# JokerJohn/Cloud_Map_Evaluation

Measured on AMD Instinct MI355X. Metric: Mpts/sec full metric suite (CD+MME+AWD) on 50M-pt pair, higher is better.
Workload: dtype f64

## Files before the change

cloud_map_evaluation_amd/csrc/me_api.hip:

```cpp
#include <cmath>
#include <cstring>

#include "me_internal.hpp"
#include "me_stat.hpp"

static std::string g_create_error;

hipEvent_t me_ctx::get_event() {
    if (!event_pool.empty()) {
        hipEvent_t e = event_pool.back();
        event_pool.pop_back();
        return e;
    }
    hipEvent_t e = nullptr;
    (void) hipEventCreate(&e);
    return e;
}

void me_ctx::timer_begin(const char *name) {
    if (!timers_on) return;
    Pending p;
    p.name = name;
    p.a = get_event();
    p.b = get_event();
// ... 26 lines not shown
__global__ void __launch_bounds__(64) k_mail(const unsigned char *__restrict__ src, unsigned char *__restrict__ dst, unsigned int bytes) {
    if (((reinterpret_cast<size_t>(src) | reinterpret_cast<size_t>(dst) | bytes) & 7u) == 0) {
        for (unsigned int i = threadIdx.x; i < bytes / 8; i += 64)
            reinterpret_cast<unsigned long long *>(dst)[i] = reinterpret_cast<const unsigned long long *>(src)[i];
    } else {
        for (unsigned int i = threadIdx.x; i < bytes; i += 64) dst[i] = src[i];
    }
}

int copy_h2d(me_ctx *ctx, void *dst_device, const void *src_host, size_t bytes) {
    if (bytes == 0) return ME_OK;
    ME_CHECK(ctx, hipMemcpyAsync(dst_device, src_host, bytes, hipMemcpyHostToDevice, ctx->stream));
    return ME_OK;
}

int copy_d2h(me_ctx *ctx, void *dst_host, const void *src_device, size_t bytes) {
    if (bytes == 0) return ME_OK;
    ME_CHECK(ctx, hipMemcpyAsync(dst_host, src_device, bytes, hipMemcpyDeviceToHost, ctx->stream));
    ME_CHECK(ctx, hipStreamSynchronize(ctx->stream));
    return ME_OK;
}

int mail_post(me_ctx *ctx, void *host_dst, const void *dev_src, size_t bytes) {
    if (bytes == 0) return ME_OK;
    if (!ctx->mail_h) {
        void *h = nullptr, *d = nullptr;
        ME_CHECK(ctx, hipHostMalloc(&h, kMailBytes, hipHostMallocMapped));
        ME_CHECK(ctx, hipHostGetDevicePointer(&d, h, 0));
        ctx->mail_h = static_cast<unsigned char *>(h);
        ctx->mail_d = static_cast<unsigned char *>(d);
    }
    const size_t off = (ctx->mail_used + 15) & ~(size_t) 15;
    if (off + bytes > kMailBytes) return copy_d2h(ctx, host_dst, dev_src, bytes);
    hipLaunchKernelGGL(k_mail, dim3(1), dim3(64), 0, ctx->stream, static_cast<const unsigned char *>(dev_src), ctx->mail_d + off,
                       (unsigned int) bytes);
    ctx->mail_pending.push_back({host_dst, off, bytes});
    ctx->mail_used = off + bytes;
    return ME_OK;
}

int mail_sync(me_ctx *ctx) {
    const hipError_t e = hipStreamSynchronize(ctx->stream);
    if (e == hipSuccess)
        for (const auto &m : ctx->mail_pending) std::memcpy(m.host, ctx->mail_h + m.off, m.bytes);
    ctx->mail_pending.clear();
    ctx->mail_used = 0;
    ME_CHECK(ctx, e);
    return ME_OK;
}

void mail_drop(me_ctx *ctx) {
    ctx->mail_pending.clear();
    ctx->mail_used = 0;
}

int need_single_gpu_cloud(me_ctx *ctx, int slot, const char *who) {
    if (slot < 0 || slot > 1) return ctx->fail(ME_ERR_ARG, std::string(who) + ": bad slot");
    Cloud &c = ctx->cloud[slot];
    if (ctx->shard_world != 1 || ctx->slab.axis >= 0 || c.slab.axis >= 0)
        return ctx->fail(ME_ERR_ARG, std::string(who) + ": single GPU only (no slab or shard mode)");
    if (!c.uploaded) return ctx->fail(ME_ERR_STATE, std::string(who) + ": cloud not uploaded");
    return ME_OK;
}
}

extern "C" {

int me_version(void) { return 100; }

static int stream_priority_for(bool main_lane) {
    int least = 0, greatest = 0;
    (void) hipDeviceGetStreamPriorityRange(&least, &greatest);
    return main_lane ? greatest : least;
}

me_ctx *me_create(int device, int flags) {
    int count = 0;
    hipError_t e = hipGetDeviceCount(&count);
    if (e != hipSuccess || count <= 0) {
        g_create_error = std::string("me_create: no HIP device available (") + hipGetErrorString(e) +
                         "); libmapeval_hip has no CPU fallback";
        return nullptr;
    }
    if (device < 0 || device >= count) {
        g_create_error = "me_create: device ordinal out of range";
        return nullptr;
    }
    e = hipSetDevice(device);
    if (e != hipSuccess) {
        g_create_error = std::string("me_create: hipSetDevice: ") + hipGetErrorString(e);
        return nullptr;
    }
    me_ctx *ctx = new me_ctx();
    ctx->device = device;
    ctx->borrow_device_input = (flags & ME_FLAG_BORROW_DEVICE_INPUT) != 0;
    ctx->morton_order = (flags & ME_FLAG_MORTON_ORDER) != 0;
    e = hipStreamCreateWithPriority(&ctx->stream, hipStreamNonBlocking, stream_priority_for(true));
    if (e != hipSuccess) {
        g_create_error = std::string("me_create: hipStreamCreate: ") + hipGetErrorString(e);
        delete ctx;
        return nullptr;
    }
    return ctx;
}

me_ctx *me_twin(me_ctx *ctx) {
    if (!ctx) return nullptr;
    if (ctx->is_twin) return ctx;
    if (ctx->twin) return ctx->twin;
    if (hipSetDevice(ctx->device) != hipSuccess) {
        ctx->fail(ME_ERR_HIP, "me_twin: hipSetDevice failed");
        return nullptr;
    }
    me_ctx *t = new me_ctx();
    t->device = ctx->device;
    t->is_twin = true;
    t->cloud.p[0] = ctx->cloud.p[0];
    t->cloud.p[1] = ctx->cloud.p[1];
    t->shard_rank = ctx->shard_rank;
    t->shard_world = ctx->shard_world;
    t->borrow_device_input = ctx->borrow_device_input;
    t->morton_order = ctx->morton_order;
    t->slab = ctx->slab;
    t->vox_hint = ctx->vox_hint;
    if (hipStreamCreateWithPriority(&t->stream, hipStreamNonBlocking, stream_priority_for(false)) != hipSuccess) {
        delete t;
        ctx->fail(ME_ERR_HIP, "me_twin: hipStreamCreate failed");
        return nullptr;
    }
    ctx->twin = t;
    return t;
}

void me_destroy(me_ctx *ctx) {
    if (!ctx) return;
    if (ctx->is_twin) return;
    if (ctx->suite_worker && ctx->suite_worker_free) {
        ctx->suite_worker_free(ctx->suite_worker);
        ctx->suite_worker = nullptr;
    }
    if (ctx->twin) {
        me_ctx *t = ctx->twin;
        ctx->twin = nullptr;
        t->is_twin = false;
        me_destroy(t);
    }
    (void) hipSetDevice(ctx->device);
    (void) hipStreamSynchronize(ctx->stream);
    for (auto &p : ctx->pending) {
        (void) hipEventDestroy(p.a);
        (void) hipEventDestroy(p.b);
    }
    for (auto e : ctx->event_pool) (void) hipEventDestroy(e);
    if (ctx->suite_event) (void) hipEventDestroy(static_cast<hipEvent_t>(ctx->suite_event));
    if (ctx->stream) (void) hipStreamDestroy(ctx->stream);
    if (ctx->mail_h) (void) hipHostFree(ctx->mail_h);
    delete ctx;
}

const char *me_last_error(me_ctx *ctx) { return ctx ? ctx->err.c_str() : g_create_error.c_str(); }

int me_set_shard(me_ctx *ctx, int rank, int world) {
    if (!ctx) return ME_ERR_ARG;
    if (world < 1 || rank < 0 || rank >= world) return ctx->fail(ME_ERR_ARG, "me_set_shard: need 0 <= rank < world");
    ctx->shard_rank = rank;
    ctx->shard_world = world;
    if (ctx->twin) {
        ctx->twin->shard_rank = rank;
        ctx->twin->shard_world = world;
    }
    return ME_OK;
}

int me_upload_cloud(me_ctx *ctx, int slot, const double *xyz_host, int64_t n, const double *T, double cell_size) {
    if (!ctx) return ME_ERR_ARG;
    return me::cloud_upload(ctx, slot, xyz_host, false, n, T, cell_size);
}

int me_upload_cloud_device(me_ctx *ctx, int slot, const double *xyz_device, int64_t n, const double *T, double cell_size) {
    if (!ctx) return ME_ERR_ARG;
    return me::cloud_upload(ctx, slot, xyz_device, true, n, T, cell_size);
}

int me_upload_slab_device(me_ctx *ctx, int slot, const double *xyz_device, int64_t n, double cell_size) {
    if (!ctx) return ME_ERR_ARG;
    if (ctx->slab.axis < 0) return ctx->fail(ME_ERR_STATE, "me_upload_slab_device: call me_set_slab first");
    return me::cloud_upload(ctx, slot, xyz_device, true, n, nullptr, cell_size, true);
}

int64_t me_cloud_size(me_ctx *ctx, int slot) {
    if (!ctx || slot < 0 || slot > 1 || !ctx->cloud[slot].uploaded) return -1;
    return ctx->cloud[slot].n;
}

int me_download_cloud(me_ctx *ctx, int slot, double *xyz_host) {
    if (!ctx) return ME_ERR_ARG;
    if (slot < 0 || slot > 1 || !xyz_host) return ctx->fail(ME_ERR_ARG, "me_download_cloud: bad argument");
    me::Cloud &c = ctx->cloud[slot];
    if (!c.uploaded) return ctx->fail(ME_ERR_STATE, "cloud not uploaded");
    ME_CHECK(ctx, hipSetDevice(ctx->device));
    ME_TRY(me::copy_d2h(ctx, xyz_host, c.xyz.p, (size_t) c.n * 24));
    ME_CHECK(ctx, hipStreamSynchronize(ctx->stream));
    return ME_OK;
}

int me_voxel_downsample(me_ctx *ctx, int slot, double voxel_size, int64_t *n_out) {
    if (!ctx) return ME_ERR_ARG;
    long long n = 0;
// ... 556 lines not shown
```

cloud_map_evaluation_amd/csrc/me_index.hip:

```cpp
#include <cmath>
#include <cstdlib>
#include <cstring>

#include "me_internal.hpp"
#include "me_vox_rows.hpp"

namespace me {

struct Mat4 {
    double m[16];
};

__global__ void k_transform(double *__restrict__ xyz, long long n, Mat4 T) {
    const long long i = (long long) blockIdx.x * blockDim.x + threadIdx.x;
    if (i >= n) return;
    const double x = xyz[3 * i], y = xyz[3 * i + 1], z = xyz[3 * i + 2];
    double h[4];
#pragma unroll
    for (int r = 0; r < 4; ++r) h[r] = ((T.m[4 * r] * x + T.m[4 * r + 1] * y) + T.m[4 * r + 2] * z) + T.m[4 * r + 3];
    xyz[3 * i] = h[0] / h[3];
    xyz[3 * i + 1] = h[1] / h[3];
    xyz[3 * i + 2] = h[2] / h[3];
}

// ... 727 lines not shown
    int L = 0;
    long long off = 0;
    for (int k = nn_shift; k <= kMortonBits; ++k) {
        if (L >= kMaxLevels) return ctx->fail(ME_ERR_ARG, "octree deeper than the level table (cloud extent / cell size too large)");
        v.count[L] = c.level_unique[k];
        v.off[L] = off;
        off += v.count[L] + 1;
        ++L;
        if (c.level_unique[k] == 1) break;
    }
    v.n_levels = L;
    ME_CHECK(ctx, c.oct_nodes.ensure((size_t) (off + kFan) * sizeof(ONode)));
    ME_CHECK(ctx, hipMemsetAsync(c.oct_nodes.as<ONode>() + off, 0, kFan * sizeof(ONode), ctx->stream));
    ME_CHECK(ctx, c.oct_pbegin.ensure((size_t) (off + kFan + 1) * 4));
    ME_CHECK(ctx, hipMemsetAsync(c.oct_pbegin.as<unsigned int>() + off, 0, (kFan + 1) * 4, ctx->stream));
    v.nodes = c.oct_nodes.as<ONode>();
    v.pbegin = c.oct_pbegin.as<unsigned int>();
    ONode *nodes = c.oct_nodes.as<ONode>();
    unsigned int *pbeg = c.oct_pbegin.as<unsigned int>();
    hipLaunchKernelGGL(k_oct_leaves, dim3(blocks_of((v.count[0] + 1) * 8)), dim3(256), 0, ctx->stream, c.sp.as<SPoint>(),
                       c.nn_grid.cell_start, v.count[0], n, nodes, pbeg);
    DevBuf &ca = ctx->tmp[2], &cb = ctx->tmp[3], &pos = ctx->tmp[1], &begin = ctx->tmp[4];
    const unsigned long long *cur = c.nn_grid.cell_code;
    for (int l = 0; l + 1 < L; ++l) {
        const long long nc = v.count[l], np = v.count[l + 1];
        if (nc <= kOctTopMax) {
            ME_CHECK(ctx, begin.ensure((size_t) (np + 1) * 4));
            ME_CHECK(ctx, ca.ensure((size_t) np * 8));
            ME_CHECK(ctx, cb.ensure((size_t) np * 8));
            unsigned long long *first = (cur == ca.as<unsigned long long>()) ? cb.as<unsigned long long>() : ca.as<unsigned long long>();
            unsigned long long *second = (first == ca.as<unsigned long long>()) ? cb.as<unsigned long long>() : ca.as<unsigned long long>();
            if (small_top)
                hipLaunchKernelGGL((k_oct_top<256>), dim3(1), dim3(256), 0, ctx->stream, nodes, pbeg, v, l, cur, first, second,
                                   begin.as<unsigned int>());
            else
                hipLaunchKernelGGL((k_oct_top<1024>), dim3(1), dim3(1024), 0, ctx->stream, nodes, pbeg, v, l, cur, first, second,
                                   begin.as<unsigned int>());
            break;
        }
        ME_CHECK(ctx, pos.ensure((size_t) nc * 4));
        ME_CHECK(ctx, begin.ensure((size_t) (np + 1) * 4));
        DevBuf &nxt = (l % 2 == 0) ? ca : cb;
        ME_CHECK(ctx, nxt.ensure((size_t) np * 8));
        ME_TRY(cell_start_ranks(ctx, cur, nc, 3, pos.as<unsigned int>()));
        hipLaunchKernelGGL(k_cell_scatter, dim3(blocks_of(nc)), dim3(256), 0, ctx->stream, cur, pos.as<unsigned int>(), nc, 3,
                           nxt.as<unsigned long long>(), begin.as<unsigned int>());
        hipLaunchKernelGGL(k_oct_up, dim3(blocks_of(np + 1)), dim3(256), 0, ctx->stream, nodes + v.off[l], nc,
                           begin.as<unsigned int>(), np, nodes + v.off[l + 1], pbeg + v.off[l], pbeg + v.off[l + 1]);
        cur = nxt.as<unsigned long long>();
    }
    return ME_OK;
}

int cloud_build_index(me_ctx *ctx, int slot, double cell_size) {
    Cloud &c = ctx->cloud[slot];
    ME_TRACE_POINT(ctx, slot == 0 ? "cloud_build_index(est): enter" : "cloud_build_index(gt): enter");
    if (!c.uploaded) return ctx->fail(ME_ERR_STATE, "cloud not uploaded");
    ME_CHECK(ctx, hipSetDevice(ctx->device));
    c.cell_size_req = cell_size;
    const long long n = c.n;
    double extent = 0;
    for (int d = 0; d < 3; ++d) extent = std::fmax(extent, c.bbox_hi[d] - c.bbox_lo[d]);
    if (!(cell_size > 0)) cell_size = (extent > 0 ? extent / 128.0 : 1.0);
    const double cell_h = cell_size * (1.0 + 0x1p-20);
    for (int d = 0; d < 3; ++d) c.origin[d] = std::floor(c.bbox_lo[d] / cell_h) * cell_h;
    extent = 0;
    for (int d = 0; d < 3; ++d) extent = std::fmax(extent, c.bbox_hi[d] - c.origin[d]);
    const double ncell = std::floor(extent / cell_h) + 1.0;
    int bits_cell = 1;
    while ((double) (1LL << bits_cell) < ncell && bits_cell <= kMortonBits) ++bits_cell;
    if (bits_cell > kMortonBits)
        return ctx->fail(ME_ERR_ARG, "cell size too small for the cloud extent (needs > 2^21 cells per axis)");
    c.shift = kMortonBits - bits_cell;
    c.cell_h = cell_h;
    c.fine_h = std::ldexp(cell_h, -c.shift);
    c.index_valid = false;
    c.mme_have = false;
    c.lg_have = false;
#ifdef ME_AB
    c.mme_feat_valid = false;
#endif
    c.nn_ref_slot = -1;
    ctx->cloud[1 - slot].nn_ref_slot = -1;

    DevBuf &codes_in = ctx->tmp[0], &iota = ctx->tmp[1], &perm = ctx->tmp[2];
    ME_CHECK(ctx, codes_in.ensure((size_t) n * 8));
    ME_CHECK(ctx, iota.ensure((size_t) n * 4));
    ME_CHECK(ctx, perm.ensure((size_t) n * 4));
    ME_CHECK(ctx, c.codes.ensure((size_t) n * 8));
    ME_CHECK(ctx, c.sp.ensure((size_t) n * sizeof(SPoint)));
    constexpr int sort_depth = ME_TUNE_SORT_DEPTH;
    const int hilbert = ctx->morton_order ? 0 : 1;
    int idx_bits = 1;
    while ((1LL << idx_bits) < n) ++idx_bits;
    constexpr int pack_allowed = ME_TUNE_SORT_PACK;
    int sort_min_level = std::max(0, c.shift - std::max(0, sort_depth));
    int pack_bits = 0;
    const bool pairs_hinted = c.sort_pairs_hint && c.hint_n == n && c.hint_shift == c.shift && c.hint_cell_h == cell_h;
    if (!pairs_hinted) c.sort_pairs_hint = false;
    if (pack_allowed && !pairs_hinted) {
        const int lvl_max = std::max(sort_min_level, c.shift - std::min(std::max(0, sort_depth), 1));
        int lvl = sort_min_level;
        while (lvl < lvl_max && 3 * (kMortonBits - lvl) + idx_bits > 64) ++lvl;
        if (3 * (kMortonBits - lvl) + idx_bits <= 64) {
            sort_min_level = lvl;
            pack_bits = idx_bits;
        }
    }
    const bool depth_cut = pack_bits > 0 && sort_min_level > std::max(0, c.shift - std::max(0, sort_depth));
#ifdef ME_DBG_INDEX
    std::fprintf(stderr, "[index slot %d] n=%lld cell_h=%.17g origin=(%.17g %.17g %.17g) bbox_lo=(%.17g %.17g %.17g) shift=%d sort_min_level=%d pack_bits=%d hinted=%d\n", slot, n, cell_h,
                 c.origin[0], c.origin[1], c.origin[2], c.bbox_lo[0], c.bbox_lo[1], c.bbox_lo[2], c.shift, sort_min_level, pack_bits, (int) pairs_hinted);
#endif
    if (pack_bits > 0) ME_CHECK(ctx, perm.ensure((size_t) n * 8));
    {
        TimerScope ts(ctx, "morton");
        hipLaunchKernelGGL(k_morton, dim3(blocks_of(n)), dim3(256), 0, ctx->stream, c.xyz.as<double>(), n, c.origin[0],
                           c.origin[1], c.origin[2], c.fine_h, sort_min_level, hilbert, pack_bits, codes_in.as<unsigned long long>(),
                           iota.as<unsigned int>());
    }
    if (pack_bits > 0)
        ME_TRY(sort_keys_u64(ctx, codes_in.as<unsigned long long>(), perm.as<unsigned long long>(), n, pack_bits,
                             pack_bits + 3 * (kMortonBits - sort_min_level)));
    else
        ME_TRY(sort_pairs_u64_u32(ctx, codes_in.as<unsigned long long>(), c.codes.as<unsigned long long>(),
                                  iota.as<unsigned int>(), perm.as<unsigned int>(), n, 3 * sort_min_level, 63));
    if (ctx->sort_hook) ctx->sort_hook(ctx->sort_hook_arg, ctx->stream);
    VoxPack vp{};
    c.vox_rec_valid = false;
    const bool fuse_vox = ME_TUNE_VOX_ONEPASS && ctx->vox_hint > 0 && vox_make_pack(c, ctx->vox_hint, n, vp);
    const long long rec_cap = vox_record_capacity(n);
    if (fuse_vox) {
        ME_CHECK(ctx, c.vox_rec_key.ensure((size_t) rec_cap * 8));
        ME_CHECK(ctx, c.vox_rec_n.ensure((size_t) rec_cap * 4));
        ME_CHECK(ctx, c.vox_rec_s.ensure((size_t) rec_cap * 8 * kVoxRec));
        ME_CHECK(ctx, c.vox_rec_cnt.ensure(kVoxCounterBytes));
        ME_CHECK(ctx, hipMemsetAsync(c.vox_rec_key.p, 0xFF, (size_t) rec_cap * 8, ctx->stream));
        ME_CHECK(ctx, hipMemsetAsync(c.vox_rec_cnt.p, 0, kVoxCounterBytes, ctx->stream));
    }
    {
        TimerScope ts(ctx, "gather");
#define ME_LAUNCH_GATHER(VOX_, PER_)                                                                                                     \
    hipLaunchKernelGGL((k_gather<VOX_, PER_>), dim3(blocks_of(n, 256 * PER_)), dim3(256), 0, ctx->stream, c.xyz.as<double>(),            \
                       pack_bits > 0 ? (const unsigned int *) nullptr : perm.as<unsigned int>(),                                       \
                       pack_bits > 0 ? perm.as<unsigned long long>() : (const unsigned long long *) nullptr,                           \
                       pack_bits > 0 ? ((1ULL << pack_bits) - 1ULL) : 0ULL, n, c.origin[0], c.origin[1], c.origin[2], c.fine_h,        \
                       c.sp.as<SPoint>(), c.codes.as<unsigned long long>(), vp, c.slab, c.vox_rec_key.as<unsigned long long>(),        \
                       c.vox_rec_n.as<int>(), c.vox_rec_s.as<double>(), c.vox_rec_cnt.as<unsigned int>(), (unsigned int) ((n + 63) / 64), \
                       (unsigned int) vox_region_size(n))
        if (fuse_vox) ME_LAUNCH_GATHER(true, kGatherPerVox);
        else ME_LAUNCH_GATHER(false, kGatherPer);
#undef ME_LAUNCH_GATHER
    }
    if (fuse_vox) {
        c.vox_rec_valid = true;
        c.vox_rec_cap = rec_cap;
        c.vox_rec_pack = vp;
    }
    {
        TimerScope ts(ctx, "cells");
        const int nblk = (int) ((n + kCellChunk - 1) / kCellChunk);
        ME_CHECK(ctx, ctx->red.ensure(64 * 8 + (size_t) (nblk + 2) * 4 * (2 + kHistLevels)));
        unsigned long long *d_hist = ctx->red.as<unsigned long long>();
        unsigned int *d_boff = reinterpret_cast<unsigned int *>(d_hist + 64), *d_bcnt = d_boff + (nblk + 2), *d_bhist = d_bcnt + (nblk + 2);
        ME_CHECK(ctx, hipMemsetAsync(d_hist, 0, 32 * 8, ctx->stream));
        hipLaunchKernelGGL(k_level_hist_rows, dim3((unsigned int) nblk), dim3(256), 0, ctx->stream, c.codes.as<unsigned long long>(), n, d_bhist);
        hipLaunchKernelGGL(k_block_counts<true>, dim3(blocks_of(nblk + 1)), dim3(256), 0, ctx->stream, d_bhist, nblk, c.shift, d_bcnt, d_hist);
        ME_TRY(exclusive_scan_u32(ctx, d_bcnt, d_boff, nblk + 1));
        unsigned long long h_hist[32];
        {
            MailGuard mg(ctx);
            ME_TRY(mail_post(ctx, h_hist, d_hist, sizeof(h_hist)));
            ME_TRY(mg.sync());
        }
        long long acc = 1;
        for (int k = kMortonBits; k >= 0; --k) {
            if (k < kMortonBits) acc += (long long) h_hist[k];
            c.level_unique[k] = (k == kMortonBits) ? 1 : acc;
        }
        int nn_shift = kMortonBits - 1;
        constexpr double nn_occ = ME_TUNE_NN_OCC;
        for (int k = sort_min_level; k < kMortonBits; ++k)
            if ((double) n / (double) c.level_unique[k] >= nn_occ) {
                nn_shift = k;
                break;
            }
        if (depth_cut && nn_shift == sort_min_level) {
            c.sort_pairs_hint = true;
            c.hint_n = n;
            c.hint_shift = c.shift;
            c.hint_cell_h = cell_h;
            ts.end();
            return cloud_build_index(ctx, slot, c.cell_size_req);
        }
        ME_TRY(build_grid_table_counted(ctx, c, c.shift, c.grid_tab, c.grid, nblk, d_bhist, d_boff, true));
        c.n_mid = 0;
        if (nn_shift == c.shift) {
            c.nn_grid = c.grid;
        } else {
            ME_TRY(build_grid_table_counted(ctx, c, nn_shift, c.nn_tab, c.nn_grid, nblk, d_bhist, d_boff, false));
            for (int k = nn_shift + 1; k < c.shift && c.n_mid < Cloud::kMaxMid; ++k) {
                ME_TRY(build_grid_table_counted(ctx, c, k, c.mid_tab[c.n_mid], c.mid_grid[c.n_mid], nblk, d_bhist, d_boff, false));
                ++c.n_mid;
            }
        }
        c.oct_deferred = false;
        c.oct_nn_shift = nn_shift;
        ts.end();
        int oct_levels = 1;
        for (int k = nn_shift; k < kMortonBits && c.level_unique[k] != 1; ++k) ++oct_levels;
        if (ctx->defer_octree || oct_levels > kMaxLevels) {
            c.oct_deferred = true;
        } else {
            TimerScope to(ctx, "octree");
            ME_TRY(build_octree(ctx, c, nn_shift, ctx->is_twin));
        }
    }
    ME_CHECK(ctx, hipGetLastError());
    ME_CHECK(ctx, hipStreamSynchronize(ctx->stream));
    c.index_valid = true;
    ME_TRACE_POINT(ctx, "cloud_build_index: done (host side)");
    return ME_OK;
}

int cloud_finish_octree(me_ctx *ctx, int slot) {
    Cloud &c = ctx->cloud[slot];
    if (!c.oct_deferred || !c.index_valid) return ME_OK;
    ME_CHECK(ctx, hipSetDevice(ctx->device));
    {
        TimerScope ts(ctx, "octree");
        ME_TRY(build_octree(ctx, c, c.oct_nn_shift, true));
    }
    ME_CHECK(ctx, hipGetLastError());
    ME_CHECK(ctx, hipStreamSynchronize(ctx->stream));
    c.oct_deferred = false;
    return ME_OK;
}

__global__ void k_slab_points(const double *__restrict__ xyz, long long n, SlabView s, const int *__restrict__ orig,
                              long long *__restrict__ orig_out, unsigned char *__restrict__ owned_out) {
    const long long i = (long long) blockIdx.x * blockDim.x + threadIdx.x;
    if (i >= n) return;
    if (orig_out) orig_out[i] = orig ? (long long) orig[i] : i;
    if (owned_out) owned_out[i] = slab_owned(s, xyz[3 * i], xyz[3 * i + 1], xyz[3 * i + 2]) ? 1 : 0;
}

int slab_points(me_ctx *ctx, int slot, int64_t *orig_index, uint8_t *owned, long long capacity, long long *count) {
    if (slot < 0 || slot > 1 || !count) return ctx->fail(ME_ERR_ARG, "me_slab_points: bad argument");
    Cloud &c = ctx->cloud[slot];
    if (!c.uploaded) return ctx->fail(ME_ERR_STATE, "me_slab_points: cloud not uploaded");
    *count = c.n;
    if ((!orig_index && !owned) || c.n == 0) return ME_OK;
    if (capacity < c.n) return ctx->fail(ME_ERR_CAPACITY, "me_slab_points: capacity too small (count returned)");
    ME_CHECK(ctx, hipSetDevice(ctx->device));
    DevBuf &oi = ctx->tmp[0], &ow = ctx->tmp[1];
    ME_CHECK(ctx, oi.ensure((size_t) c.n * 8));
    ME_CHECK(ctx, ow.ensure((size_t) c.n));
    hipLaunchKernelGGL(k_slab_points, dim3(blocks_of(c.n)), dim3(256), 0, ctx->stream, c.xyz.as<double>(), c.n, c.slab,
                       c.slab_identity ? (const int *) nullptr : c.slab_orig.as<int>(), orig_index ? oi.as<long long>() : nullptr,
                       owned ? ow.as<unsigned char>() : nullptr);
    if (orig_index) ME_TRY(copy_d2h(ctx, orig_index, oi.p, (size_t) c.n * 8));
    if (owned) ME_TRY(copy_d2h(ctx, owned, ow.p, (size_t) c.n));
    ME_CHECK(ctx, hipStreamSynchronize(ctx->stream));
    return ME_OK;
}

}
```

cloud_map_evaluation_amd/csrc/me_internal.hpp:

```cpp
#pragma once

#include <hip/hip_runtime.h>

#include <algorithm>
#include <cstdint>
#include <cstdlib>
#include <cstdio>
#include <map>
#include <string>
#include <vector>

#include "../../include/mapeval_hip.h"

namespace me {

constexpr int kFan = 8;
constexpr int kMaxLevels = 17;
constexpr int kMortonBits = 21;

struct DevBuf {
    void *p = nullptr;
    size_t bytes = 0;
    bool owned = true;
    ~DevBuf() { release(); }
// ... 161 lines not shown
    int mme_fx_scale = 0;
#endif
    DevBuf vox_tmp;
    DevBuf vox_key;
    DevBuf vox_n;
    DevBuf vox_mu;
    DevBuf vox_sigma;
    DevBuf vox_entropy;
    DevBuf normals;
    DevBuf cov;
    bool have_normals = false, have_cov = false;
    DevBuf fpfh;
    bool fpfh_valid = false;
    DevBuf outlier_keep;
    bool outlier_keep_valid = false;
    DevBuf cluster_labels, cluster_sizes;
    long long cluster_n = 0;
    bool cluster_valid = false;
    DevBuf lg_eig, lg_k, lg_val;
    bool lg_have = false;
    DevBuf plane_labels;
    std::vector<me_plane_record> plane_rec;
    bool plane_valid = false;
    unsigned long long lg_serial = 0, plane_serial = 0;
    DevBuf mom_axis;
    bool mom_have = false;
    DevBuf surf_e, surf_c;
    bool surf_have = false;
    unsigned long long mom_lg_serial = 0, mom_plane_serial = 0;
};

struct TimerRec {
    double total_ms = 0;
    long long launches = 0;
};

}

struct me_ctx {
    int device = 0;
    hipStream_t stream = nullptr;
    std::string err;
    me::Cloud own_cloud[2];
    struct CloudSet {
        me::Cloud *p[2];
        me::Cloud &operator[](int i) const { return *p[i]; }
    } cloud;
    me_ctx *twin = nullptr;
    void (*sort_hook)(void *arg, hipStream_t stream) = nullptr;
    void *sort_hook_arg = nullptr;
    void *suite_event = nullptr;
    void *suite_worker = nullptr;
    void (*suite_worker_free)(void *) = nullptr;
    unsigned char *mail_h = nullptr, *mail_d = nullptr;
    size_t mail_used = 0;
    struct MailItem {
        void *host;
        size_t off, bytes;
    };
    std::vector<MailItem> mail_pending;
    bool is_twin = false;
    me_ctx() {
        cloud.p[0] = &own_cloud[0];
        cloud.p[1] = &own_cloud[1];
    }
    me::DevBuf tmp[6];
    me::DevBuf red;
    void *host_pinned = nullptr;
    size_t host_pinned_bytes = 0;
    int shard_rank = 0, shard_world = 1;
    bool borrow_device_input = false;
    bool morton_order = false;
    me::SlabView slab{-1, 0, 0, 0, 0};
    bool defer_octree = false;
    double vox_hint = 0;
    bool timers_on = false;
    std::map<std::string, me::TimerRec> timers;
    struct Pending {
        std::string name;
        hipEvent_t a, b;
    };
    std::vector<Pending> pending;
    std::vector<hipEvent_t> event_pool;
    long long nn_fallback = 0, nn_queries = 0;
    long long mme_pairs = 0;
    me::DevBuf mme_pairs_buf;
    me::DevBuf mme_refine;
    long long mme_refined = 0;
    me::DevBuf nn_far;
    me::DevBuf nn_flags, nn_list_a, nn_list_b;
    me::DevBuf mme_keep_e, mme_keep_v;
    long long mme_keep_n = -1;
    me::DevBuf outlier_tmp[2];
    me::DevBuf cluster_tmp[5];
    me::DevBuf mom_tmp[3];
    me::DevBuf rs_tmp[4];
    long long rs_compact[2] = {0, 0};
    me::DevBuf plane_tmp[7];
    me::DevBuf nn1_dbg_buf;
    unsigned long long *nn1_dbg() {
        if (!nn1_dbg_buf.p) {
            if (nn1_dbg_buf.ensure(128) != hipSuccess) return nullptr;
            (void) hipMemsetAsync(nn1_dbg_buf.p, 0, 128, stream);
        }
        return nn1_dbg_buf.as<unsigned long long>();
    }
// ... 50 lines not shown
        open = false;
    }
    ~TimerScope() { end(); }
};

#ifndef ME_TUNE_XCD_CHUNK
#define ME_TUNE_XCD_CHUNK 128
#endif
#ifndef ME_TUNE_SORT_DEPTH
#define ME_TUNE_SORT_DEPTH 2
#endif
#ifndef ME_TUNE_SORT_PACK
#define ME_TUNE_SORT_PACK 1
#endif
#ifndef ME_TUNE_NN_OCC
#define ME_TUNE_NN_OCC 6.0
#endif
#ifndef ME_TUNE_MME_LEADER_ORIGIN
#define ME_TUNE_MME_LEADER_ORIGIN 1
#endif
#ifndef ME_TUNE_NN_SGPR_MASKS
#define ME_TUNE_NN_SGPR_MASKS 1
#endif
#ifndef ME_TUNE_NN1_FAR_CAP
#define ME_TUNE_NN1_FAR_CAP 64
#endif
#ifndef ME_TUNE_NN_FAR_LEAF
#define ME_TUNE_NN_FAR_LEAF 1024
#endif
#ifndef ME_TUNE_MME_WAVES
#define ME_TUNE_MME_WAVES 8
#endif
#ifndef ME_TUNE_MME_REFINE_COND
#define ME_TUNE_MME_REFINE_COND 1.8e-6
#endif
#ifndef ME_TUNE_SUITE_SORT_FIRST
#define ME_TUNE_SUITE_SORT_FIRST 1
#endif
#ifndef ME_TUNE_VOX_MERGE_SORT
#define ME_TUNE_VOX_MERGE_SORT 1
#endif
#ifndef ME_TUNE_VOX_ONEPASS
#define ME_TUNE_VOX_ONEPASS 1
#endif
#ifndef ME_TUNE_SUITE_DEFER_OCTREE
#define ME_TUNE_SUITE_DEFER_OCTREE 1
#endif
#ifndef ME_TUNE_SUITE_VOX_EARLY
#define ME_TUNE_SUITE_VOX_EARLY 1
#endif
#ifndef ME_TUNE_SUITE_NN_FIRST
#define ME_TUNE_SUITE_NN_FIRST 1
#endif
inline unsigned int xcd_chunk_setting() { return (unsigned int) ME_TUNE_XCD_CHUNK; }
inline unsigned int blocks_of(long long n, int block = 256) { return (unsigned int) std::max<long long>(1, (n + block - 1) / block); }

int copy_h2d(me_ctx *ctx, void *dst_device, const void *src_host, size_t bytes);
int copy_d2h(me_ctx *ctx, void *dst_host, const void *src_device, size_t bytes);
constexpr size_t kMailBytes = 128 * 1024;
int mail_post(me_ctx *ctx, void *host_dst, const void *dev_src, size_t bytes);
int mail_sync(me_ctx *ctx);
void mail_drop(me_ctx *ctx);
int need_single_gpu_cloud(me_ctx *ctx, int slot, const char *who);
struct MailGuard {
    me_ctx *c;
    bool armed = true;
    explicit MailGuard(me_ctx *ctx) : c(ctx) {}
    int sync() {
        armed = false;
        return mail_sync(c);
    }
    ~MailGuard() {
        if (armed) mail_drop(c);
    }
};

int sort_pairs_u64_u32(me_ctx *ctx, const unsigned long long *k_in, unsigned long long *k_out,
                       const unsigned int *v_in, unsigned int *v_out, long long n, int begin_bit, int end_bit);
int sort_pairs_merge_u64_u32(me_ctx *ctx, const unsigned long long *k_in, unsigned long long *k_out, const unsigned int *v_in,
                             unsigned int *v_out, long long n);
int exclusive_scan_u32(me_ctx *ctx, const unsigned int *in, unsigned int *out, long long n);
int exclusive_scan_u32_plain(me_ctx *ctx, const unsigned int *in, unsigned int *out, long long n);
int cell_start_ranks(me_ctx *ctx, const unsigned long long *codes, long long n, int shift3, unsigned int *out);
int sort_keys_f64(me_ctx *ctx, const double *in, double *out, long long n);
int sort_keys_u64(me_ctx *ctx, const unsigned long long *in, unsigned long long *out, long long n, int begin_bit, int end_bit);
int select_flagged_u32(me_ctx *ctx, const unsigned char *flags, long long n, unsigned int *out, unsigned int *count_device);

int cloud_upload(me_ctx *ctx, int slot, const double *src, bool src_on_device, long long n, const double *T,
                 double cell_size, bool prefiltered = false);
int cloud_build_index(me_ctx *ctx, int slot, double cell_size);
int cloud_finish_octree(me_ctx *ctx, int slot);
int cloud_finish(me_ctx *ctx, int slot, bool bbox_ready = false);
void cloud_reset_replaced(me_ctx *ctx, int slot, long long n, double cell_size_req);
int cloud_transform(me_ctx *ctx, int slot, const double *T);
int voxel_downsample(me_ctx *ctx, int slot, double voxel_size, long long *n_out);
int voxel_downsample_into(me_ctx *src_ctx, int src_slot, me_ctx *dst_ctx, int dst_slot, double voxel_size, long long *n_out);

int perturb_cloud(me_ctx *ctx, int dst_slot, int src_slot, const me_perturb_params *p, long long *n_out);
int fpfh(me_ctx *ctx, int slot, const me_fpfh_params *p, double *features_host);
int fpfh_match(me_ctx *ctx, int src_slot, int ref_slot, int mutual, int32_t *corr_host, long long *n_corr);
int global_register(me_ctx *ctx, int src_slot, int ref_slot, const me_globreg_params *p, double T_out[16], me_globreg_info *info,
                    int64_t *scores);
int statistical_outlier(me_ctx *ctx, int slot, int nb_neighbors, double std_ratio, double *avg_host, uint8_t *keep_host,
                        me_outlier_info *info);
int radius_outlier(me_ctx *ctx, int slot, int nb_points, double radius, int32_t *counts_host, uint8_t *keep_host, me_outlier_info *info);
int outlier_select_into(me_ctx *src_ctx, int src_slot, me_ctx *dst_ctx, int dst_slot, long long *n_out);
int local_geometry(me_ctx *ctx, int slot, double radius, int min_k, me_local_geom_out *out);
int local_geometry_fetch(me_ctx *ctx, int slot, double *eig_host, int32_t *k_host, uint8_t *valid_host);
int radius_normals(me_ctx *ctx, int slot, double radius, int min_k, const double *viewpoint, int invalid_z, me_radius_normals_out *out);
int nn_surface_error(me_ctx *ctx, int qslot, const me_surface_params *p, me_surface_out *out);
int nn_surface_fetch(me_ctx *ctx, int qslot, double *plane_d_host, double *cos_n_host);
int segment_planes(me_ctx *ctx, int slot, const me_plane_params *p, me_plane_record *planes_host, int32_t *labels_host, int64_t *scores_host,
                   me_plane_info *info);
int plane_fetch(me_ctx *ctx, int slot, me_plane_record *planes_host, long long capacity, long long *n_planes, int32_t *labels_host);
int plane_keep(me_ctx *ctx, int slot, int plane, int invert, uint8_t *keep_host, me_outlier_info *info);
// ... 469 lines not shown
```

cloud_map_evaluation_amd/csrc/me_suite.hip:

```cpp
#include <atomic>
#include <chrono>
#include <condition_variable>
#include <cstring>
#include <exception>
#include <mutex>
#include <new>
#include <thread>

#include "me_internal.hpp"

namespace {

using Clock = std::chrono::steady_clock;
inline double ms_since(Clock::time_point t0) { return std::chrono::duration<double, std::milli>(Clock::now() - t0).count(); }

bool is_identity(const double *T) {
    if (!T) return true;
    for (int i = 0; i < 16; ++i)
        if (T[i] != ((i % 5 == 0) ? 1.0 : 0.0)) return false;
    return true;
}

struct SuiteLane {
    me_ctx *t = nullptr;
    const me_suite_params *p = nullptr;
    const double *gt = nullptr;
    long long n_gt = 0;
    bool gt_on_device = false, upload_gt = false, wait_for_link = false, pin_gt = false;
    bool est_voxel_on_main = false;
    std::atomic<int> est_voxel_taken{0};
    bool gt_pinned = false;
    std::mutex m;
    std::condition_variable cv;
    bool est_on_device = false;
    bool est_final = false;
    bool gt_ready = false;
    bool aborted = false;
    std::atomic<int> rc{ME_OK};
    bool finished = false;
    bool started = false;
    me_nn_partial back{};
    double back_sig[5] = {0, 0, 0, 0, 0};
    bool est_tree = false;
    bool gt_tree = false;
    bool tables_ready = false;
    hipEvent_t sort_event = nullptr;
    bool sort_queued = false;
    static void sort_hook(void *self, hipStream_t stream) {
        SuiteLane *l = static_cast<SuiteLane *>(self);
        if (l->sort_event && !l->sort_queued) {
            (void) hipEventRecord(l->sort_event, stream);
            l->set(&SuiteLane::sort_queued);
        }
    }

    void set(bool SuiteLane::*flag) {
        {
            std::lock_guard<std::mutex> g(m);
            this->*flag = true;
        }
        cv.notify_all();
    }
    bool is_set(bool SuiteLane::*flag) {
        std::lock_guard<std::mutex> g(m);
        return this->*flag;
    }
    bool wait(bool SuiteLane::*flag) {
        std::unique_lock<std::mutex> g(m);
        cv.wait(g, [&] { return this->*flag || aborted; });
        return !aborted;
    }
    void run() {
        int r;
        try {
            r = body();
        } catch (const std::bad_alloc &) {
            r = t->fail(ME_ERR_HIP, "me_run_suite_from: out of host memory on the second lane");
        } catch (const std::exception &e) {
            r = t->fail(ME_ERR_HIP, std::string("me_run_suite_from: second lane: ") + e.what());
        }
        rc = r;
        {
            std::lock_guard<std::mutex> g(m);
            gt_ready = true;
            gt_tree = true;
            sort_queued = true;
            finished = true;
        }
        cv.notify_all();
    }
    int body() {
        if (hipSetDevice(t->device) != hipSuccess) return t->fail(ME_ERR_HIP, "me_run_suite_from: hipSetDevice failed on the second lane");
        if (upload_gt) {
            if (pin_gt) {
                gt_pinned = hipHostRegister(const_cast<double *>(gt), (size_t) n_gt * 24, hipHostRegisterDefault) == hipSuccess;
                (void) hipGetLastError();
            }
            if (wait_for_link && !wait(&SuiteLane::est_on_device)) return ME_OK;
            t->sort_hook = sort_event ? &SuiteLane::sort_hook : nullptr;
            t->sort_hook_arg = this;
            const int urc = me::cloud_upload(t, ME_SLOT_GT, gt, gt_on_device, n_gt, nullptr, p->nn_radius);
            t->sort_hook = nullptr;
            if (urc != ME_OK) return urc;
        }
        set(&SuiteLane::sort_queued);
        set(&SuiteLane::gt_ready);
        ME_TRY(me::cloud_finish_octree(t, ME_SLOT_GT));
        set(&SuiteLane::gt_tree);
#if ME_TUNE_SUITE_NN_FIRST
        bool gt_table = false;
#if ME_TUNE_SUITE_VOX_EARLY
        if (t->cloud[ME_SLOT_GT].vox_rec_valid) {
            ME_TRY(me::voxel_build(t, ME_SLOT_GT, p->vmd_voxel_size, false));
            gt_table = true;
        }
#endif
        if (!wait(&SuiteLane::est_final)) return ME_OK;
#if ME_TUNE_SUITE_VOX_EARLY
        if (gt_table && !est_voxel_on_main && t->cloud[ME_SLOT_EST].vox_rec_valid && !est_voxel_taken.exchange(1)) {
            ME_TRY(me::voxel_build(t, ME_SLOT_EST, p->vmd_voxel_size, false));
            set(&SuiteLane::tables_ready);
        }
#endif
        if (!wait(&SuiteLane::est_tree)) return ME_OK;
        ME_TRY(me::nn_search(t, ME_SLOT_GT, ME_SLOT_EST));
        ME_TRY(me::nn_partial(t, ME_SLOT_GT, p->icp_max_distance, p->gate_mode, p->trunc, &back));
        ME_TRY(back_sigma());
        if (!gt_table) ME_TRY(me::voxel_build(t, ME_SLOT_GT, p->vmd_voxel_size, false));
        if (!est_voxel_on_main && !est_voxel_taken.exchange(1)) ME_TRY(me::voxel_build(t, ME_SLOT_EST, p->vmd_voxel_size, false));
#else
        ME_TRY(me::voxel_build(t, ME_SLOT_GT, p->vmd_voxel_size, false));
        if (!wait(&SuiteLane::est_final)) return ME_OK;
        if (!est_voxel_on_main) ME_TRY(me::voxel_build(t, ME_SLOT_EST, p->vmd_voxel_size, false));
        if (!wait(&SuiteLane::est_tree)) return ME_OK;
        ME_TRY(me::nn_search(t, ME_SLOT_GT, ME_SLOT_EST));
        ME_TRY(me::nn_partial(t, ME_SLOT_GT, p->icp_max_distance, p->gate_mode, p->trunc, &back));
        ME_TRY(back_sigma());
#endif
        return ME_OK;
    }
    int back_sigma() {
        double mean[5];
        for (int k = 0; k < 5; ++k) mean[k] = back.sum_d[k] / (double) back.n_corr;
        return me::nn_sigma(t, ME_SLOT_GT, p->icp_max_distance, p->gate_mode, mean, back_sig);
    }
    bool join() {
        if (started) {
            std::unique_lock<std::mutex> g(m);
            cv.wait(g, [&] { return finished; });
        }
        return rc.load() == ME_OK;
    }
    void abort_and_join() {
        {
            std::lock_guard<std::mutex> g(m);
            aborted = true;
        }
        cv.notify_all();
        (void) join();
    }
    ~SuiteLane() { abort_and_join(); }
};

struct LaneWorker {
    std::mutex m;
    std::condition_variable cv;
    SuiteLane *job = nullptr;
    bool quit = false;
    std::thread th;
    void loop() {
        for (;;) {
            SuiteLane *j = nullptr;
            {
                std::unique_lock<std::mutex> g(m);
                cv.wait(g, [&] { return job != nullptr || quit; });
                if (quit) return;
                j = job;
                job = nullptr;
            }
            j->run();
        }
    }
    void post(SuiteLane *j) {
        {
            std::lock_guard<std::mutex> g(m);
            job = j;
// ... 116 lines not shown
        me_ctx *a, *b = nullptr;
        bool defer;
        double keep_a, keep_b = 0;
        VoxHint(me_ctx *c, double v, bool d) : a(c), defer(d), keep_a(c->vox_hint) {
            a->vox_hint = v;
            a->defer_octree = d;
        }
        void also(me_ctx *t, double v) {
            b = t;
            if (b) {
                keep_b = keep_a;
                b->vox_hint = v;
                b->defer_octree = defer;
            }
        }
        ~VoxHint() {
            a->vox_hint = keep_a;
            a->defer_octree = false;
            if (b) {
                b->vox_hint = keep_b;
                b->defer_octree = false;
            }
        }
    } vox_hint(ctx, upload ? p->vmd_voxel_size : 0.0, ME_TUNE_SUITE_DEFER_OCTREE && upload && p->evaluate_mme);

    if (!upload) {
        for (int slot = 0; slot < 2; ++slot) {
            const me::Cloud &c = ctx->cloud[slot];
            if (c.n > 0 && !index_fits_radius(c, p->nn_radius)) ME_TRY(me::cloud_build_index(ctx, slot, p->nn_radius));
        }
    }
    SuiteLane lane;
    LaneWorker *worker = nullptr;
    if (overlap) {
        lane.t = me_twin(ctx);
        if (!lane.t) return ME_ERR_HIP;
        vox_hint.also(lane.t, upload ? p->vmd_voxel_size : 0.0);
        worker = lane_worker(ctx);
        if (!worker) return ME_ERR_HIP;
        lane.p = p;
        lane.gt = gt;
        lane.n_gt = n_gt;
        lane.gt_on_device = on_device;
        lane.upload_gt = upload;
        lane.wait_for_link = upload && !on_device;
        lane.pin_gt = pin;
        lane.est_voxel_on_main = upload && !on_device;
#if ME_TUNE_SUITE_SORT_FIRST
        if (upload && on_device && p->evaluate_mme) {
            if (!ctx->suite_event) ME_CHECK(ctx, hipEventCreateWithFlags(reinterpret_cast<hipEvent_t *>(&ctx->suite_event), hipEventDisableTiming));
            lane.sort_event = static_cast<hipEvent_t>(ctx->suite_event);
        }
#endif
        worker->post(&lane);
    }
    bool est_pinned = false, gt_pinned_here = false;
    auto main_lane = [&]() -> int {
        auto t0 = Clock::now();
        if (upload) {
            if (pin) est_pinned = hipHostRegister(const_cast<double *>(est), (size_t) n_est * 24, hipHostRegisterDefault) == hipSuccess;
            if (pin && !overlap) gt_pinned_here = hipHostRegister(const_cast<double *>(gt), (size_t) n_gt * 24, hipHostRegisterDefault) == hipSuccess;
            (void) hipGetLastError();
            ME_TRY(me::cloud_upload(ctx, ME_SLOT_EST, est, on_device, n_est, nullptr, p->nn_radius));
            if (overlap) lane.set(&SuiteLane::est_on_device);
            if (!overlap) ME_TRY(me::cloud_upload(ctx, ME_SLOT_GT, gt, on_device, n_gt, nullptr, p->nn_radius));
        } else if (overlap) {
            lane.set(&SuiteLane::est_on_device);
        }
        out->stage_ms[0] = ms_since(t0);
        if (overlap && !moved) lane.set(&SuiteLane::est_final);
        if (p->evaluate_mme) {
            double s = 0;
            long long nv = 0;
            t0 = Clock::now();
            if (overlap && lane.sort_event) {
                if (!lane.wait(&SuiteLane::sort_queued)) return lane.rc.load() != ME_OK ? lane.rc.load() : ME_ERR_STATE;
                ME_CHECK(ctx, hipStreamWaitEvent(ctx->stream, lane.sort_event, 0));
            }
            ME_TRY(me::mme_run(ctx, ME_SLOT_EST, p->nn_radius, 10, nullptr, nullptr, &s, &nv));
            out->stage_ms[4] = ms_since(t0);
            out->mme_est = nv > 0 ? s / (double) nv : 0.0;
            out->mme_est_valid = nv;
        }
        if (moved) {
            t0 = Clock::now();
            if (p->evaluate_mme) ME_TRY(me::mme_carry_out(ctx, ME_SLOT_EST));
            ME_TRY(me::cloud_transform(ctx, ME_SLOT_EST, T));
            if (p->evaluate_mme) ME_TRY(me::mme_carry_in(ctx, ME_SLOT_EST));
            out->stage_ms[0] += ms_since(t0);
            if (overlap) lane.set(&SuiteLane::est_final);
        }
        ME_TRY(me::cloud_finish_octree(ctx, ME_SLOT_EST));
        if (overlap) lane.set(&SuiteLane::est_tree);
        if (overlap && upload && !on_device) {
            t0 = Clock::now();
            ME_TRY(me::voxel_build(ctx, ME_SLOT_EST, p->vmd_voxel_size, false));
            out->stage_ms[6] += ms_since(t0);
        }
        if (overlap) {
            lane.wait(&SuiteLane::gt_ready);
            if (lane.rc.load() != ME_OK) return lane.rc.load();
        }
        if (p->evaluate_mme && p->evaluate_gt_mme) {
            double s = 0;
            long long nv = 0;
            t0 = Clock::now();
            ME_TRY(me::mme_run(ctx, ME_SLOT_GT, p->nn_radius, 5, nullptr, nullptr, &s, &nv));
            out->stage_ms[5] = ms_since(t0);
            out->mme_gt = nv > 0 ? s / (double) nv : 0.0;
            out->mme_gt_valid = nv;
        }
        me_nn_partial pe{}, pg{};
        t0 = Clock::now();
        if (overlap) {
            lane.wait(&SuiteLane::gt_tree);
            if (lane.rc.load() != ME_OK) return lane.rc.load();
        } else {
            ME_TRY(me::cloud_finish_octree(ctx, ME_SLOT_GT));
        }
        ME_TRY(me::nn_search(ctx, ME_SLOT_EST, ME_SLOT_GT));
        ME_TRY(me::nn_partial(ctx, ME_SLOT_EST, p->icp_max_distance, p->gate_mode, p->trunc, &pe));
        out->stage_ms[1] = ms_since(t0);
        t0 = Clock::now();
#if ME_TUNE_SUITE_NN_FIRST
        if (overlap && !lane.est_voxel_on_main && !lane.est_voxel_taken.exchange(1)) {
            ME_TRY(me::voxel_build(ctx, ME_SLOT_EST, p->vmd_voxel_size, false));
            out->stage_ms[6] += ms_since(t0);
            t0 = Clock::now();
        }
#endif
        double sig_e[5], sig_g[5];
        ME_TRY(sigma_pass(ctx, ME_SLOT_EST, p, pe, sig_e));
        out->stage_ms[3] = ms_since(t0);
        int64_t n_rows = 0;
        bool vmd_done = false;
        auto vmd = [&]() -> int {
            const auto tv = Clock::now();
            ME_TRY(me_awd_scs(ctx, p->vmd_voxel_size, p->min_pts > 0 ? p->min_pts : 100, p->scs_radius > 0 ? p->scs_radius : 5, nullptr,
                              nullptr, &n_rows, &out->awd, &out->scs, nullptr));
            out->stage_ms[6] += ms_since(tv);
            vmd_done = true;
            return ME_OK;
        };
        if (overlap && lane.is_set(&SuiteLane::tables_ready)) ME_TRY(vmd());
        t0 = Clock::now();
        if (overlap) {
            if (!lane.join()) return lane.rc.load();
            pg = lane.back;
            for (int k = 0; k < 5; ++k) sig_g[k] = lane.back_sig[k];
        } else {
            ME_TRY(me::nn_search(ctx, ME_SLOT_GT, ME_SLOT_EST));
            ME_TRY(me::nn_partial(ctx, ME_SLOT_GT, p->icp_max_distance, p->gate_mode, p->trunc, &pg));
            ME_TRY(sigma_pass(ctx, ME_SLOT_GT, p, pg, sig_g));
        }
        out->stage_ms[2] = ms_since(t0);
        me_nn_finalize(&pe, sig_e, ctx->cloud[ME_SLOT_EST].n, &out->est_gt);
        me_nn_finalize(&pg, sig_g, ctx->cloud[ME_SLOT_GT].n, &out->gt_est);
        out->full_chamfer = out->est_gt.mean_nn_dist + out->gt_est.mean_nn_dist;
        if (!vmd_done) ME_TRY(vmd());
        out->n_w_voxels = n_rows;
        return ME_OK;
    };
    int rc;
    try {
        rc = main_lane();
    } catch (const std::bad_alloc &) {
        rc = ctx->fail(ME_ERR_HIP, "me_run_suite_from: out of host memory");
    } catch (const std::exception &e) {
        rc = ctx->fail(ME_ERR_HIP, std::string("me_run_suite_from: ") + e.what());
// ... 13 lines not shown
```

Baseline: 2257.

## Run GT index tail on high-priority stream and move est octree to worker lane

Adds a high-priority tail stream. During the two-lane suite, the post-sort part of the ground-truth index build is redirected to that stream so it can compete with the main lane's MME kernels. When tail priority is on, the est-octree finish also moves from the main thread to the worker lane, with new flags to order the hand-off. The aim is to shorten the critical path and fill the gap between the two MME kernels. The cost is extra cross-stream synchronisation and more complex lane ordering, with some risk of deadlock or ordering bugs.

New measurement: 2317 (median of 6 runs). 1.03x the previous value.

```diff
diff --git a/cloud_map_evaluation_amd/csrc/me_api.hip b/cloud_map_evaluation_amd/csrc/me_api.hip
--- a/cloud_map_evaluation_amd/csrc/me_api.hip
+++ b/cloud_map_evaluation_amd/csrc/me_api.hip
@@ -102,6 +102,17 @@
 void mail_drop(me_ctx *ctx) {
     ctx->mail_pending.clear();
     ctx->mail_used = 0;
+}
+
+int tail_stream_ensure(me_ctx *ctx) {
+    if (ctx->tail_stream) return ME_OK;
+    ME_CHECK(ctx, hipSetDevice(ctx->device));
+    for (void *&ev : ctx->tail_event)
+        if (!ev) ME_CHECK(ctx, hipEventCreateWithFlags(reinterpret_cast<hipEvent_t *>(&ev), hipEventDisableTiming));
+    int least = 0, greatest = 0;
+    (void) hipDeviceGetStreamPriorityRange(&least, &greatest);
+    ME_CHECK(ctx, hipStreamCreateWithPriority(&ctx->tail_stream, hipStreamNonBlocking, greatest));
+    return ME_OK;
 }
 
 int need_single_gpu_cloud(me_ctx *ctx, int slot, const char *who) {
@@ -204,6 +215,12 @@
     for (auto e : ctx->event_pool) (void) hipEventDestroy(e);
     if (ctx->suite_event) (void) hipEventDestroy(static_cast<hipEvent_t>(ctx->suite_event));
     if (ctx->stream) (void) hipStreamDestroy(ctx->stream);
+    if (ctx->tail_stream) {
+        (void) hipStreamSynchronize(ctx->tail_stream);
+        (void) hipStreamDestroy(ctx->tail_stream);
+    }
+    for (void *ev : ctx->tail_event)
+        if (ev) (void) hipEventDestroy(static_cast<hipEvent_t>(ev));
     if (ctx->mail_h) (void) hipHostFree(ctx->mail_h);
     delete ctx;
 }
diff --git a/cloud_map_evaluation_amd/csrc/me_index.hip b/cloud_map_evaluation_amd/csrc/me_index.hip
--- a/cloud_map_evaluation_amd/csrc/me_index.hip
+++ b/cloud_map_evaluation_amd/csrc/me_index.hip
@@ -803,6 +803,37 @@
     return ME_OK;
 }
 
+struct IndexTail {
+    me_ctx *c;
+    hipStream_t home = nullptr;
+    bool on = false;
+    explicit IndexTail(me_ctx *ctx) : c(ctx) {}
+    int begin() {
+        if (!c->index_tail || !c->tail_stream) return ME_OK;
+        ME_CHECK(c, hipEventRecord(static_cast<hipEvent_t>(c->tail_event[0]), c->stream));
+        ME_CHECK(c, hipStreamWaitEvent(c->tail_stream, static_cast<hipEvent_t>(c->tail_event[0]), 0));
+        home = c->stream;
+        c->stream = c->tail_stream;
+        on = true;
+        return ME_OK;
+    }
+    int end() {
+        if (!on) return ME_OK;
+        on = false;
+        hipStream_t tail = c->stream;
+        c->stream = home;
+        ME_CHECK(c, hipEventRecord(static_cast<hipEvent_t>(c->tail_event[1]), tail));
+        ME_CHECK(c, hipStreamWaitEvent(home, static_cast<hipEvent_t>(c->tail_event[1]), 0));
+        return ME_OK;
+    }
+    ~IndexTail() {
+        if (on) {
+            (void) hipStreamSynchronize(c->stream);
+            (void) end();
+        }
+    }
+};
+
 int cloud_build_index(me_ctx *ctx, int slot, double cell_size) {
     Cloud &c = ctx->cloud[slot];
     ME_TRACE_POINT(ctx, slot == 0 ? "cloud_build_index(est): enter" : "cloud_build_index(gt): enter");
@@ -877,6 +908,8 @@
         ME_TRY(sort_pairs_u64_u32(ctx, codes_in.as<unsigned long long>(), c.codes.as<unsigned long long>(),
                                   iota.as<unsigned int>(), perm.as<unsigned int>(), n, 3 * sort_min_level, 63));
     if (ctx->sort_hook) ctx->sort_hook(ctx->sort_hook_arg, ctx->stream);
+    IndexTail tail(ctx);
+    ME_TRY(tail.begin());
     VoxPack vp{};
     c.vox_rec_valid = false;
     const bool fuse_vox = ME_TUNE_VOX_ONEPASS && ctx->vox_hint > 0 && vox_make_pack(c, ctx->vox_hint, n, vp);
@@ -942,6 +975,7 @@
             c.hint_shift = c.shift;
             c.hint_cell_h = cell_h;
             ts.end();
+            ME_TRY(tail.end());
             return cloud_build_index(ctx, slot, c.cell_size_req);
         }
         ME_TRY(build_grid_table_counted(ctx, c, c.shift, c.grid_tab, c.grid, nblk, d_bhist, d_boff, true));
@@ -969,6 +1003,7 @@
     }
     ME_CHECK(ctx, hipGetLastError());
     ME_CHECK(ctx, hipStreamSynchronize(ctx->stream));
+    ME_TRY(tail.end());
     c.index_valid = true;
     ME_TRACE_POINT(ctx, "cloud_build_index: done (host side)");
     return ME_OK;
diff --git a/cloud_map_evaluation_amd/csrc/me_internal.hpp b/cloud_map_evaluation_amd/csrc/me_internal.hpp
--- a/cloud_map_evaluation_amd/csrc/me_internal.hpp
+++ b/cloud_map_evaluation_amd/csrc/me_internal.hpp
@@ -237,6 +237,9 @@
     void *suite_event = nullptr;
     void *suite_worker = nullptr;
     void (*suite_worker_free)(void *) = nullptr;
+    hipStream_t tail_stream = nullptr;
+    void *tail_event[2] = {nullptr, nullptr};
+    bool index_tail = false;
     unsigned char *mail_h = nullptr, *mail_d = nullptr;
     size_t mail_used = 0;
     struct MailItem {
@@ -393,6 +396,9 @@
 #ifndef ME_TUNE_SUITE_NN_FIRST
 #define ME_TUNE_SUITE_NN_FIRST 1
 #endif
+#ifndef ME_TUNE_SUITE_GT_TAIL_PRIO
+#define ME_TUNE_SUITE_GT_TAIL_PRIO 2
+#endif
 inline unsigned int xcd_chunk_setting() { return (unsigned int) ME_TUNE_XCD_CHUNK; }
 inline unsigned int blocks_of(long long n, int block = 256) { return (unsigned int) std::max<long long>(1, (n + block - 1) / block); }
 
@@ -402,6 +408,7 @@
 int mail_post(me_ctx *ctx, void *host_dst, const void *dev_src, size_t bytes);
 int mail_sync(me_ctx *ctx);
 void mail_drop(me_ctx *ctx);
+int tail_stream_ensure(me_ctx *ctx);
 int need_single_gpu_cloud(me_ctx *ctx, int slot, const char *who);
 struct MailGuard {
     me_ctx *c;
diff --git a/cloud_map_evaluation_amd/csrc/me_suite.hip b/cloud_map_evaluation_amd/csrc/me_suite.hip
--- a/cloud_map_evaluation_amd/csrc/me_suite.hip
+++ b/cloud_map_evaluation_amd/csrc/me_suite.hip
@@ -46,6 +46,8 @@
     bool tables_ready = false;
     hipEvent_t sort_event = nullptr;
     bool sort_queued = false;
+    bool tail_prio = false;
+    bool est_mme_done = false;
     static void sort_hook(void *self, hipStream_t stream) {
         SuiteLane *l = static_cast<SuiteLane *>(self);
         if (l->sort_event && !l->sort_queued) {
@@ -84,6 +86,7 @@
             std::lock_guard<std::mutex> g(m);
             gt_ready = true;
             gt_tree = true;
+            if (tail_prio) est_tree = true;
             sort_queued = true;
             finished = true;
         }
@@ -99,8 +102,10 @@
             if (wait_for_link && !wait(&SuiteLane::est_on_device)) return ME_OK;
             t->sort_hook = sort_event ? &SuiteLane::sort_hook : nullptr;
             t->sort_hook_arg = this;
+            t->index_tail = tail_prio;
             const int urc = me::cloud_upload(t, ME_SLOT_GT, gt, gt_on_device, n_gt, nullptr, p->nn_radius);
             t->sort_hook = nullptr;
+            t->index_tail = false;
             if (urc != ME_OK) return urc;
         }
         set(&SuiteLane::sort_queued);
@@ -116,6 +121,10 @@
         }
 #endif
         if (!wait(&SuiteLane::est_final)) return ME_OK;
+        if (tail_prio) {
+            ME_TRY(me::cloud_finish_octree(t, ME_SLOT_EST));
+            set(&SuiteLane::est_tree);
+        }
 #if ME_TUNE_SUITE_VOX_EARLY
         if (gt_table && !est_voxel_on_main && t->cloud[ME_SLOT_EST].vox_rec_valid && !est_voxel_taken.exchange(1)) {
             ME_TRY(me::voxel_build(t, ME_SLOT_EST, p->vmd_voxel_size, false));
@@ -123,6 +132,9 @@
         }
 #endif
         if (!wait(&SuiteLane::est_tree)) return ME_OK;
+#if ME_TUNE_SUITE_GT_TAIL_PRIO == 1
+        if (tail_prio && !wait(&SuiteLane::est_mme_done)) return ME_OK;
+#endif
         ME_TRY(me::nn_search(t, ME_SLOT_GT, ME_SLOT_EST));
         ME_TRY(me::nn_partial(t, ME_SLOT_GT, p->icp_max_distance, p->gate_mode, p->trunc, &back));
         ME_TRY(back_sigma());
@@ -132,6 +144,10 @@
         ME_TRY(me::voxel_build(t, ME_SLOT_GT, p->vmd_voxel_size, false));
         if (!wait(&SuiteLane::est_final)) return ME_OK;
         if (!est_voxel_on_main) ME_TRY(me::voxel_build(t, ME_SLOT_EST, p->vmd_voxel_size, false));
+        if (tail_prio) {
+            ME_TRY(me::cloud_finish_octree(t, ME_SLOT_EST));
+            set(&SuiteLane::est_tree);
+        }
         if (!wait(&SuiteLane::est_tree)) return ME_OK;
         ME_TRY(me::nn_search(t, ME_SLOT_GT, ME_SLOT_EST));
         ME_TRY(me::nn_partial(t, ME_SLOT_GT, p->icp_max_distance, p->gate_mode, p->trunc, &back));
@@ -354,6 +370,15 @@
             lane.sort_event = static_cast<hipEvent_t>(ctx->suite_event);
         }
 #endif
+#if ME_TUNE_SUITE_GT_TAIL_PRIO
+        if (upload && on_device && p->evaluate_mme) {
+            if (me::tail_stream_ensure(lane.t) != ME_OK) {
+                ctx->err = lane.t->err;
+                return ME_ERR_HIP;
+            }
+            lane.tail_prio = true;
+        }
+#endif
         worker->post(&lane);
     }
     bool est_pinned = false, gt_pinned_here = false;
@@ -384,6 +409,7 @@
             out->mme_est = nv > 0 ? s / (double) nv : 0.0;
             out->mme_est_valid = nv;
         }
+        if (overlap) lane.set(&SuiteLane::est_mme_done);
         if (moved) {
             t0 = Clock::now();
             if (p->evaluate_mme) ME_TRY(me::mme_carry_out(ctx, ME_SLOT_EST));
@@ -392,8 +418,10 @@
             out->stage_ms[0] += ms_since(t0);
             if (overlap) lane.set(&SuiteLane::est_final);
         }
-        ME_TRY(me::cloud_finish_octree(ctx, ME_SLOT_EST));
-        if (overlap) lane.set(&SuiteLane::est_tree);
+        if (!(overlap && lane.tail_prio)) {
+            ME_TRY(me::cloud_finish_octree(ctx, ME_SLOT_EST));
+            if (overlap) lane.set(&SuiteLane::est_tree);
+        }
         if (overlap && upload && !on_device) {
             t0 = Clock::now();
             ME_TRY(me::voxel_build(ctx, ME_SLOT_EST, p->vmd_voxel_size, false));
@@ -417,6 +445,10 @@
         if (overlap) {
             lane.wait(&SuiteLane::gt_tree);
             if (lane.rc.load() != ME_OK) return lane.rc.load();
+            if (lane.tail_prio) {
+                lane.wait(&SuiteLane::est_tree);
+                if (lane.rc.load() != ME_OK) return lane.rc.load();
+            }
         } else {
             ME_TRY(me::cloud_finish_octree(ctx, ME_SLOT_GT));
         }
diff --git a/profiles/timeline_lanes.py b/profiles/timeline_lanes.py
--- /dev/null
+++ b/profiles/timeline_lanes.py
@@ -0,0 +1,40 @@
+import csv
+import glob
+import re
+import sys
+
+rows = []
+for f in glob.glob(sys.argv[1] + "/**/*kernel_trace.csv", recursive=True):
+    with open(f) as fh:
+        for r in csv.DictReader(fh):
+            n = re.sub(r"\(.*", "", r["Kernel_Name"])
+            n = re.sub(r"<.*", "", n).split("::")[-1].split(" ")[-1]
+            rows.append((int(r["Start_Timestamp"]), int(r["End_Timestamp"]), r.get("Queue_Id", "?"), n))
+rows.sort()
+mort = [i for i, r in enumerate(rows) if r[3] == "k_morton"]
+step = rows[mort[-2]:]
+t0 = step[0][0]
+ms = lambda t: (t - t0) / 1e6
+print("two-lane step: %.2f ms wall, %d kernels" % (ms(max(r[1] for r in step)), len(step)))
+queues = sorted({r[2] for r in step}, key=lambda q: min(r[0] for r in step if r[2] == q))
+for q in queues:
+    ks = [r for r in step if r[2] == q]
+    print("--- queue %s: %d kernels, busy %.2f ms; kernels > 0.08 ms (start, duration)" % (q, len(ks), sum(r[1] - r[0] for r in ks) / 1e6))
+    for r in ks:
+        if r[1] - r[0] > 80_000:
+            print("  %7.3f  dur %7.3f  %s" % (ms(r[0]), (r[1] - r[0]) / 1e6, r[3]))
+mme = [r for r in step if r[3] == "k_mme3"]
+fill = [r for r in step if r[3] == "k_cell_fill"]
+gath = [r for r in step if r[3] == "k_gather"]
+grid = [r for r in step if r[3] == "k_nn_grid"]
+main_q = mme[0][2]
+print("--- figures (ms)")
+print("map k_mme3: %.3f -> %.3f (%.3f)" % (ms(mme[0][0]), ms(mme[0][1]), (mme[0][1] - mme[0][0]) / 1e6))
+print("ground truth k_mme3: %.3f -> %.3f (%.3f); hole between the two: %.3f" % (ms(mme[1][0]), ms(mme[1][1]), (mme[1][1] - mme[1][0]) / 1e6, (mme[1][0] - mme[0][1]) / 1e6))
+print("  kernels on the main queue inside the hole: %d" % sum(1 for r in step if r[2] == main_q and mme[0][1] <= r[0] < mme[1][0]))
+g = [r for r in gath if r[2] != main_q][-1]
+print("ground truth k_gather: %.3f -> %.3f (%.3f)" % (ms(g[0]), ms(g[1]), (g[1] - g[0]) / 1e6))
+print("ground truth's last k_cell_fill ends: %.3f" % ms(max(r[1] for r in fill if r[2] != main_q)))
+for r in grid:
+    print("k_nn_grid on queue %s (%s lane): %.3f -> %.3f (%.3f)" % (r[2], "main" if r[2] == main_q else "second", ms(r[0]), ms(r[1]), (r[1] - r[0]) / 1e6))
+print("end of the step: %.3f" % ms(max(r[1] for r in step)))
```
